# facebookresearch/visual_inertial_bundle_adjustment

Hardware: AMD Instinct MI355X
Metric: LM iterations/sec on 10k-pose/300k-landmark VI-BA (higher is better)
Workload: dtype f64; 1 GPU; config C: 5941186 obs, 300000 landmarks, 10000 rigs, reduced order 150483; rigs=10000, landmarks=300000, observations=5941186, parallelism=single GPU

## Files before the change

### visual_inertial_bundle_adjustment_amd/csrc/finalize.hip

```cpp
#include "host.hpp"

namespace viba_host {
namespace {

Knobs readKnobs(const vb_handle_s& h) {
  Knobs k;
  if (const char* e = getenv("VIBA_ND_CUTWIN")) k.cutWin = std::max(0.0, std::min(0.45, atof(e)));
  if (const char* e = getenv("VIBA_ND_LEAF")) k.leafDims = std::max<int64_t>(64, atoll(e));
  k.stats = getenv("VIBA_STATS") != nullptr;
  k.ptFuseMax = h.ptFuseMax, k.useSn = h.useSn, k.snStreams = h.snStreams;
  return k;
}

int uploadSched(const SchedHost& H, Sched& S) {
  static_cast<SchedShape&>(S) = H;
  if (upload(&S.potrfTileD, H.potrfTile) || upload(&S.potrfColD, H.potrfCol) || upload(&S.trsmDiagD, H.trsmDiag) ||
      upload(&S.trsmTargetD, H.trsmTarget) || upload(&S.trsmColD, H.trsmCol) || upload(&S.trsmRowD, H.trsmRow) ||
      upload(&S.updD, H.upd) || upload(&S.fanPairsD, H.fanPairs) || upload(&S.tasksFD, H.tasksF) ||
      upload(&S.tasksBD, H.tasksB) || upload(&S.expFD, H.expF) || upload(&S.expBD, H.expB) ||
      upload(&S.preReadyD, H.preReady) || upload(&S.ptfD, H.ptf) || upload(&S.ptfDiagD, H.ptfDiag))
    return VB_E_HIP;
  return 0;
}

int uploadSnSched(const SnSchedHost& H, SnSched& S) {
  static_cast<SnSchedShape&>(S) = H;
  if (upload(&S.updD, H.upd) || upload(&S.fanPairsD, H.fanPairs) || upload(&S.potD, H.pot) || upload(&S.rowD, H.row) ||
      upload(&S.fusD, H.fus) || upload(&S.copyD, H.copy) || upload(&S.invEarlyD, H.invEarly) ||
      upload(&S.invLateD, H.invLate))
    return VB_E_HIP;
  return 0;
}

void copyToHandle(vb_handle h, const Symbolic& A) {
  Dev& d = h->d;
  d.jac = makeJac(h->cfg.imu_calib_options);
  d.reproj = makeLoss(h->cfg.reproj_loss_radius, h->cfg.reproj_loss_cutoff);
  d.imu = makeLoss(h->cfg.imu_loss_radius, h->cfg.imu_loss_cutoff);
  d.T = TS;
  for (int k = 0; k < 9; k++) d.nvar[k] = A.reg.nvar[k];
  const int64_t nPts = A.reg.nPts;
  d.nRV = A.lay.nRV, d.nRed = A.lay.nRed, d.nPts = nPts, d.nT = A.lay.nT, d.nTiles = A.pat.nTiles;
  d.nObs = A.obs.nObs, d.nObsPad = A.obs.nObsPad, d.nYcol = A.pan.nYcol;
  d.nLxChunk = (int64_t)A.pan.lxChunk.size() / 3;
  d.lmB = A.shard.lmBegin, d.lmE = A.shard.lmEnd, d.root = A.shard.isRoot ? 1 : 0;
  d.nLmSmall = A.shard.nLmSmall, d.nLmBig = A.shard.nLmBig, d.lmBigCols = A.shard.lmBigCols;
  d.obB = A.shard.obB, d.obE = A.shard.obE, d.obFree = A.shard.obFree, d.fB = A.shard.fB, d.fE = A.shard.fE;
  d.nGroups = (int64_t)A.schur.grpRed.size() / 4;
  d.nTileWorks = (int64_t)A.schur.works.size();
  for (int fk = 1; fk < 14; fk++) {
    SmallFactors& sf = d.sf[fk];
    sf.nv = kNumVars[fk], sf.n = (int64_t)h->fint[fk].size(), sf.nc = A.small.nc[fk], sf.stage = A.small.stage[fk];
  }
  d.nSmallStage = A.small.nSmallStage;
  d.myRank = h->partRank, d.world = h->partWorld;
  d.nRS = h->nRS;

  h->rvKind = A.lay.rvKind, h->rvHandle = A.lay.rvHandle, h->rvDim = A.lay.rvDim, h->rvOff = A.lay.rvOff;
  h->lmOfPoint = A.reg.lmOfPoint;
  h->colOwner = A.lay.colOwner;
  h->nRedReal = A.lay.nRedReal, h->nParts = (int64_t)A.nd.partBegin.size();
  h->nParams = nPts + A.lay.nRV;
  h->order = nPts * 3 + A.lay.nRedReal;
  h->nPadRows = (int64_t)A.lay.padRows.size();
  h->nLmObs = A.obs.lmObs[nPts];
  h->lmBegin = A.shard.lmBegin, h->lmEnd = A.shard.lmEnd, h->isRoot = A.shard.isRoot;
  h->tileFill = A.pat.tileFill;
  h->colStart = A.pat.colStart, h->colTilesH = A.pat.colTiles, h->colRowsH = A.pat.colRows;
  h->rowStart = A.pat.rowStart, h->rowTilesH = A.pat.rowTiles, h->rowColH = A.pat.rowCol;
  h->nClear = (int64_t)A.schur.clearTiles.size();
  h->nTileEnt = (int64_t)A.schur.ents.size(), h->nObEnt = d.nGroups;
  h->tileFirst = A.schur.tileFirst, h->tileCount = A.schur.tileCount;
  h->shardTiles = A.schur.shardTiles;
  h->zeroRuns = A.part.zeroRuns, h->rootTiles = A.part.rootTiles, h->rootRows = A.part.rootRows;
  h->nOwnRows = (int64_t)A.part.ownRows.size();
  h->nLevels = A.pat.nLevels;
  h->nPairs = A.sch[0].nPairs + A.sch[1].nPairs;
  h->costRsB[0] = A.cost.rsBegin[0], h->costRsB[1] = A.cost.rsBegin[1];
  if (A.preint.present) h->piNoise = A.preint.noise;
}

int uploadRsTables(vb_handle h) {
  Dev& d = h->d;
  if (h->rsDevice) {
    const int64_t kWidenNs = 20000000;
    h->rsOff.assign(h->nRS + 1, 0);
    for (int32_t t = 0; t < h->nRS; t++) {
      const int64_t a = (h->rsMid[t] - h->rsHalf[t]) * 1000 - kWidenNs, b = (h->rsMid[t] + h->rsHalf[t]) * 1000 + kWidenNs;
      const int64_t cnt = std::upper_bound(h->imuT.begin(), h->imuT.end(), b) -
                          std::lower_bound(h->imuT.begin(), h->imuT.end(), a);
      h->rsOff[t + 1] = h->rsOff[t] + cnt + 4;
// ... 122 lines not shown
```

### visual_inertial_bundle_adjustment_amd/csrc/solver.hip

```cpp
#include "kernel_common.hpp"
#include <algorithm>
#include <string>

namespace viba {


template <int J>
__device__ __forceinline__ double rowbcast(double v) {
  return __builtin_amdgcn_mov_dpp(v, 0x150 + J, 0xF, 0xF, true);
}

__device__ __forceinline__ double rsqrt_nr(double x) {
  double y = __builtin_amdgcn_rsq(x);
  const double e = __builtin_fma(-(x * y), y, 1.0);
  return __builtin_fma(e * y, __builtin_fma(e, 0.375, 0.5), y);
}

template <int C, int J>
struct Upd16 {
  static __device__ __forceinline__ void run(double (&s)[16], double lc) {
    s[J] -= lc * rowbcast<J>(lc);
    Upd16<C, J + 1>::run(s, lc);
  }
};
template <int C>
struct Upd16<C, 16> {
  static __device__ __forceinline__ void run(double (&)[16], double) {}
};
template <int C>
struct Chol16 {
  static __device__ __forceinline__ void run(double (&s)[16], double (&invd)[16], int lane, bool& bad) {
    const double piv = rowbcast<C>(s[C]);
    bad |= !(piv > 0.0);
    const double y = rsqrt_nr(piv);
    invd[C] = y;
    const double lc = s[C] * y;
    s[C] = lc;
    Upd16<C, C + 1>::run(s, lc);
    Chol16<C + 1>::run(s, invd, lane, bad);
  }
};
template <>
struct Chol16<16> {
  static __device__ __forceinline__ void run(double (&)[16], double (&)[16], int, bool&) {}
};

template <int LDT = TS>
__device__ __forceinline__ void diag16(double* T, double* scratch, double* dinvS, int i, double4_t S, int lane,
                                       bool& bad) {
  const int lr = lane & 15, lq = lane >> 4;
#pragma unroll
  for (int r = 0; r < 4; r++) scratch[(lq + 4 * r) * 16 + lr] = S[r];
  __builtin_amdgcn_wave_barrier();
  double s[16], invd[16];
#pragma unroll
  for (int c = 0; c < 16; c++) s[c] = scratch[lr * 16 + c];
  Chol16<0>::run(s, invd, lane, bad);
  __builtin_amdgcn_wave_barrier();
  if (lane < 16) {
#pragma unroll
    for (int c = 0; c < 16; c++) {
      const double v = (c <= lane) ? s[c] : 0.0;
      scratch[lane * 16 + c] = v;
      T[(16 * i + c) * LDT + 16 * i + lane] = v;
    }
  }
  __builtin_amdgcn_fence(__ATOMIC_RELEASE, "wavefront");
  __builtin_amdgcn_wave_barrier();
  __builtin_amdgcn_fence(__ATOMIC_ACQUIRE, "wavefront");
  double acc[16];
#pragma unroll
  for (int r = 0; r < 16; r++) acc[r] = (r == lr) ? 1.0 : 0.0;
#pragma unroll
  for (int k = 0; k < 16; k++) {
    acc[k] *= invd[k];
#pragma unroll
    for (int r = k + 1; r < 16; r++) acc[r] -= scratch[r * 16 + k] * acc[k];
  }
  if (lane < 16) {
#pragma unroll
    for (int r = 0; r < 16; r++) dinvS[i * 256 + lane * 16 + r] = acc[r];
  }
  __builtin_amdgcn_wave_barrier();
}

__device__ __forceinline__ void lds_to_global(double* dst, const double* src, int n, int tid, int nthreads) {
  double* p = dst + tid;
  const double* q = src + tid;
#pragma unroll 8
  for (int i = tid; i < n; i += nthreads, p += nthreads, q += nthreads) *p = *q;
}

__device__ __forceinline__ void wave_sync_lds() {
  __builtin_amdgcn_fence(__ATOMIC_RELEASE, "wavefront");
  __builtin_amdgcn_wave_barrier();
  __builtin_amdgcn_fence(__ATOMIC_ACQUIRE, "wavefront");
}
__device__ __forceinline__ void potrf_forward(const Dev& d, const double* T, const double* dinvS, double* sh, int J,
                                              const double* bJ, double* y, int lane, bool store = true) {
  double br = bJ[lane];
#pragma unroll
  for (int i = 0; i < 4; i++) {
    sh[64 + lane] = br;
    wave_sync_lds();
    if ((lane >> 4) == i) {
      const int l = lane & 15;
      double v = 0.0;
#pragma unroll
      for (int m = 0; m < 16; m++) v += dinvS[i * 256 + m * 16 + l] * sh[64 + 16 * i + m];
      sh[16 * i + l] = v;
    }
    wave_sync_lds();
    if (i < 3) {
#pragma unroll
      for (int m = 0; m < 16; m++) br -= T[(16 * i + m) * TS + lane] * sh[16 * i + m];
    }
  }
  const int64_t row = (int64_t)J * TS + lane;
  if (store) y[row] = row < d.nRed ? sh[lane] : 0.0;
}

__device__ __forceinline__ void potrf4_core(const Dev& d, const double* A, double* T, double* scratch, double* dinvS,
                                            int tid) {
  const int lane = tid & 63, w = tid >> 6;
  const int lr = lane & 15, lq = lane >> 4;
  double4_t R[4];
#pragma unroll
  for (int j = 0; j < 4; j++) {
    if (j < w) {
#pragma unroll
      for (int r = 0; r < 4; r++) R[j][r] = A[(16 * j + lq + 4 * r) * TS + 16 * w + lr];
    } else if (j == w) {
#pragma unroll
      for (int r = 0; r < 4; r++) R[j][r] = A[(16 * w + lr) * TS + 16 * w + lq + 4 * r];
    } else {
#pragma unroll
      for (int r = 0; r < 4; r++) T[(16 * j + lq + 4 * r) * TS + 16 * w + lr] = 0.0;
    }
  }
  bool bad = false;
#pragma unroll
  for (int k = 0; k < 4; k++) {
    if (w == k) {
      diag16(T, scratch, dinvS, k, R[k], lane, bad);
    }
    __syncthreads();
    double4_t Lt = double4_t{0, 0, 0, 0};
    if (w > k) {
#pragma unroll
      for (int s = 0; s < 4; s++) Lt = mfma64(dinvS[k * 256 + (4 * s + lq) * 16 + lr], R[k][s], Lt);
#pragma unroll
      for (int r = 0; r < 4; r++) T[(16 * k + lq + 4 * r) * TS + 16 * w + lr] = Lt[r];
#pragma unroll
      for (int j = k + 1; j < 4; j++)
        if (j == w) {
#pragma unroll
          for (int s = 0; s < 4; s++) R[j] = mfma64(-Lt[s], Lt[s], R[j]);
        }
    }
    if (k < 2) {
      __syncthreads();
#pragma unroll
      for (int j = k + 1; j < 3; j++)
        if (j < w) {
#pragma unroll
          for (int s = 0; s < 4; s++) R[j] = mfma64(-T[(16 * k + 4 * s + lq) * TS + 16 * j + lr], Lt[s], R[j]);
        }
    }
  }
  __syncthreads();
  if (bad && lane == 0) atomicOr(d.err, 8);
}

__global__ void __launch_bounds__(256) potrf4_kernel(Dev d, const int32_t* tileList, const int32_t* cols,
                                                     double* dinvAll, const double* fwdB, double* fwdY) {
  __shared__ double T[TS * TS];
  __shared__ double scratch[256];
  __shared__ double dinvS[1024];
  const int tid = threadIdx.x, w = tid >> 6;
  double* A = d.tiles + (int64_t)tileList[blockIdx.x] * TS * TS;
  double* dinvG = dinvAll + (int64_t)cols[blockIdx.x] * 1024;
  potrf4_core(d, A, T, scratch, dinvS, tid);
  if (fwdB && w == 0) potrf_forward(d, T, dinvS, scratch, cols[blockIdx.x], fwdB + (int64_t)cols[blockIdx.x] * TS, fwdY, tid & 63);
  lds_to_global(A, T, TS * TS, tid, 256);
  lds_to_global(dinvG, dinvS, 1024, tid, 256);
}

__global__ void __launch_bounds__(256) potrf_trsm_kernel(Dev d, const int32_t* items, double* Lscr, double* dinvAll,
                                                         double* fwdB, double* fwdY) {
  __shared__ double T[TS * TS];
  __shared__ double scratch[256];
  __shared__ double dinvS[1024];
  const int32_t* it = items + 5 * (int64_t)blockIdx.x;
  const int32_t diagT = it[0], col = it[1], target = it[2], row = it[3], writer = it[4];
  const int tid = threadIdx.x, lane = tid & 63, w = tid >> 6;
  const int lr = lane & 15, lq = lane >> 4;
  double* At = target >= 0 ? d.tiles + (int64_t)target * TS * TS : nullptr;
  double av[4][4];
  if (At) {
#pragma unroll
    for (int k = 0; k < 4; k++)
#pragma unroll
      for (int r = 0; r < 4; r++) av[k][r] = At[(16 * k + lq + 4 * r) * TS + 16 * w + lr];
  }
  potrf4_core(d, d.tiles + (int64_t)diagT * TS * TS, T, scratch, dinvS, tid);
  if (fwdB && w == 0) potrf_forward(d, T, dinvS, scratch, col, fwdB + (int64_t)col * TS, fwdY, lane, writer != 0);
  if (writer) {
    lds_to_global(Lscr + (int64_t)col * TS * TS, T, TS * TS, tid, 256);
    lds_to_global(dinvAll + (int64_t)col * 1024, dinvS, 1024, tid, 256);
  }
  if (!At) return;
  __syncthreads();
  double4_t Xt[4];
#pragma unroll
  for (int k = 0; k < 4; k++) {
    double4_t acc = double4_t{av[k][0], av[k][1], av[k][2], av[k][3]};
#pragma unroll
    for (int k2 = 0; k2 < k; k2++)
#pragma unroll
      for (int s = 0; s < 4; s++) acc = mfma64(-T[(16 * k2 + 4 * s + lq) * TS + 16 * k + lr], Xt[k2][s], acc);
    double4_t res = double4_t{0, 0, 0, 0};
#pragma unroll
    for (int s = 0; s < 4; s++) res = mfma64(dinvS[k * 256 + (4 * s + lq) * 16 + lr], acc[s], res);
    Xt[k] = res;
  }
#pragma unroll
  for (int k = 0; k < 4; k++)
// ... 29 lines not shown
  for (int k = 0; k < 4; k++) {
    double4_t a = acc[k];
#pragma unroll
    for (int k2 = 0; k2 < k; k2++)
#pragma unroll
      for (int s = 0; s < 4; s++) a = mfma64(-lv[k * (k - 1) / 2 + k2][s], Xt[k2][s], a);
    double4_t res = double4_t{0, 0, 0, 0};
#pragma unroll
    for (int s = 0; s < 4; s++) res = mfma64(dv[k][s], a[s], res);
    Xt[k] = res;
  }
}
template <int LD = TS>
__device__ __forceinline__ void gemm_nt_sub(const double* M, const double4_t (&Xt)[4], double4_t (&acc)[4], int lr, int lq,
                                            int kmax = 3) {
#pragma unroll
  for (int k = 0; k < 4; k++) {
    if (k > kmax) break;
    double mv[4][4];
#pragma unroll
    for (int k2 = 0; k2 < 4; k2++)
#pragma unroll
      for (int s = 0; s < 4; s++) mv[k2][s] = M[(16 * k2 + 4 * s + lq) * LD + 16 * k + lr];
#pragma unroll
    for (int k2 = 0; k2 < 4; k2++)
#pragma unroll
      for (int s = 0; s < 4; s++) acc[k] = mfma64(-mv[k2][s], Xt[k2][s], acc[k]);
  }
}
__device__ __forceinline__ void load_rows(const double* A, double4_t (&acc)[4], int w, int lr, int lq) {
#pragma unroll
  for (int k = 0; k < 4; k++)
#pragma unroll
    for (int r = 0; r < 4; r++) acc[k][r] = A[(16 * k + lq + 4 * r) * TS + 16 * w + lr];
}
__device__ __forceinline__ void store_rows(double* A, const double4_t (&X)[4], int w, int lr, int lq) {
#pragma unroll
  for (int k = 0; k < 4; k++)
#pragma unroll
    for (int r = 0; r < 4; r++) A[(16 * k + lq + 4 * r) * TS + 16 * w + lr] = X[k][r];
}
__device__ __forceinline__ double rows_dot(const double4_t (&X)[4], const double* y, int lq) {
  double v = 0.0;
#pragma unroll
  for (int k = 0; k < 4; k++)
#pragma unroll
    for (int r = 0; r < 4; r++) v += X[k][r] * y[16 * k + lq + 4 * r];
  v += __shfl_xor(v, 16, 64);
  v += __shfl_xor(v, 32, 64);
  return v;
}

template <int NB, int LDT>
__device__ __forceinline__ void potrf_core(const Dev& d, const double* A11, const double* A21, const double* A22,
                                           double* T, double* scratch, double* dinvS, int tid,
                                           const double* b0 = nullptr, const double* b1 = nullptr,
                                           double* yb = nullptr) {
  const int lane = tid & 63, w = tid >> 6;
  const int lr = lane & 15, lq = lane >> 4;
  double bw = 0.0;
  if (b0 && w < NB) bw = (w < 4 ? b0 : b1)[16 * (w & 3) + lr];
  double4_t R[NB];
  if (w < NB) {
#pragma unroll
    for (int j = 0; j < NB; j++) {
      const double* P = w < 4 ? A11 : (j < 4 ? A21 : A22);
      const int rr = 16 * (w & 3), cc = 16 * (j & 3);
      if (j < w) {
#pragma unroll
        for (int r = 0; r < 4; r++) R[j][r] = P[(cc + lq + 4 * r) * TS + rr + lr];
      } else if (j == w) {
#pragma unroll
        for (int r = 0; r < 4; r++) R[j][r] = P[(cc + lr) * TS + rr + lq + 4 * r];
      } else {
#pragma unroll
        for (int r = 0; r < 4; r++) T[(16 * j + lq + 4 * r) * LDT + 16 * w + lr] = 0.0;
      }
    }
  }
  bool bad = false;
#pragma unroll
  for (int k = 0; k < NB; k++) {
    if (w == k) {
      diag16<LDT>(T, scratch, dinvS, k, R[k], lane, bad);
      if (b0) {
        if (lq == 0) yb[16 * k + lr] = bw;
        wave_sync_lds();
        if (lq == 0) {
          double v = 0.0;
#pragma unroll
          for (int m = 0; m < 16; m++) v += dinvS[k * 256 + m * 16 + lr] * yb[16 * k + m];
          yb[128 + 16 * k + lr] = v;
        }
      }
    }
    __syncthreads();
    double4_t Lt = double4_t{0, 0, 0, 0};
    if (w > k && w < NB) {
#pragma unroll
      for (int s = 0; s < 4; s++) Lt = mfma64(dinvS[k * 256 + (4 * s + lq) * 16 + lr], R[k][s], Lt);
#pragma unroll
      for (int r = 0; r < 4; r++) T[(16 * k + lq + 4 * r) * LDT + 16 * w + lr] = Lt[r];
      if (b0) {
        double v = 0.0;
#pragma unroll
        for (int r = 0; r < 4; r++) v += Lt[r] * yb[128 + 16 * k + lq + 4 * r];
        v += __shfl_xor(v, 16, 64);
        v += __shfl_xor(v, 32, 64);
        bw -= v;
      }
#pragma unroll
      for (int j = k + 1; j < NB; j++)
        if (j == w) {
#pragma unroll
          for (int s = 0; s < 4; s++) R[j] = mfma64(-Lt[s], Lt[s], R[j]);
        }
    }
    if (k < NB - 2) {
      __syncthreads();
#pragma unroll
      for (int j = k + 1; j < NB - 1; j++)
        if (j < w && w < NB) {
#pragma unroll
          for (int s = 0; s < 4; s++) R[j] = mfma64(-T[(16 * k + 4 * s + lq) * LDT + 16 * j + lr], Lt[s], R[j]);
        }
    }
  }
  __syncthreads();
  if (bad && lane == 0) atomicOr(d.err, 8);
}

template <int NB, int LDT>
__device__ __forceinline__ void trsm_lds(const double* T, const double* dinvS, const double4_t (&a)[NB], double4_t (&X)[NB],
                                         int lr, int lq) {
#pragma unroll
  for (int k = 0; k < NB; k++) {
    double4_t acc = a[k];
#pragma unroll
    for (int k2 = 0; k2 < k; k2++)
#pragma unroll
      for (int s = 0; s < 4; s++) acc = mfma64(-T[(16 * k2 + 4 * s + lq) * LDT + 16 * k + lr], X[k2][s], acc);
    double4_t res = double4_t{0, 0, 0, 0};
#pragma unroll
    for (int s = 0; s < 4; s++) res = mfma64(dinvS[k * 256 + (4 * s + lq) * 16 + lr], acc[s], res);
    X[k] = res;
  }
}

template <int NB, int LDT>
__device__ __forceinline__ void store_block_tiles(double* L11, double* L21, double* L22, const double* T, int tid,
                                                  int nthreads) {
  for (int i = tid; i < (16 * NB) * (16 * NB); i += nthreads) {
    const int col = i / (16 * NB), row = i % (16 * NB);
    if (row < 64 && col >= 64) continue;
    double* P = row < 64 ? L11 : (col < 64 ? L21 : L22);
    P[(col & 63) * TS + (row & 63)] = T[col * LDT + row];
  }
}

__global__ void __launch_bounds__(512) snpotrf8_kernel(Dev d, const int32_t* items, double* dinvAll, const double* fwdB,
                                                       double* fwdY) {
  __shared__ double T[128 * 128];
  __shared__ double scratch[256];
  __shared__ double dinvS[8 * 256];
  __shared__ double yb[256];
  const int32_t* it = items + 4 * (int64_t)blockIdx.x;
  const int32_t t11 = it[0], J = it[1], t21 = it[2], t22 = it[3];
  const int tid = threadIdx.x, lane = tid & 63, w = tid >> 6;
  double* A11 = d.tiles + (int64_t)t11 * TS * TS;
  if (t21 < 0) {
    potrf_core<4, 128>(d, A11, nullptr, nullptr, T, scratch, dinvS, tid, fwdB ? fwdB + (int64_t)J * TS : nullptr,
                       nullptr, yb);
    if (fwdB && w == 0) {
      const int64_t row = (int64_t)J * TS + lane;
      fwdY[row] = row < d.nRed ? yb[128 + lane] : 0.0;
    }
    store_block_tiles<4, 128>(A11, nullptr, nullptr, T, tid, 512);
    for (int i = tid; i < 1024; i += 512) dinvAll[(int64_t)J * 1024 + i] = dinvS[i];
    return;
  }
  double* A21 = d.tiles + (int64_t)t21 * TS * TS;
  double* A22 = d.tiles + (int64_t)t22 * TS * TS;
  potrf_core<8, 128>(d, A11, A21, A22, T, scratch, dinvS, tid, fwdB ? fwdB + (int64_t)J * TS : nullptr,
                     fwdB ? fwdB + (int64_t)(J + 1) * TS : nullptr, yb);
  if (fwdB && w < 2) {
    const int64_t row = (int64_t)(J + w) * TS + lane;
    fwdY[row] = row < d.nRed ? yb[128 + 64 * w + lane] : 0.0;
  }
  store_block_tiles<8, 128>(A11, A21, A22, T, tid, 512);
  for (int i = tid; i < 2048; i += 512) dinvAll[(int64_t)J * 1024 + i] = dinvS[i];
}

__global__ void __launch_bounds__(512) snpotrf_trsm8_kernel(Dev d, const int32_t* items, double* Lscr, double* dinvAll,
                                                            double* fwdB, double* fwdY) {
  __shared__ double T[128 * 128];
  __shared__ double scratch[256];
  __shared__ double dinvS[8 * 256];
  __shared__ double yb[256];
  const int32_t* it = items + 8 * xcd_block(blockIdx.x, gridDim.x);
  const int32_t t11 = it[0], J = it[1], t21 = it[2], t22 = it[3], tI1 = it[4], tI2 = it[5], I = it[6], writer = it[7];
  const int tid = threadIdx.x, lane = tid & 63, w = tid >> 6;
  const int lr = lane & 15, lq = lane >> 4;
  const bool two = t21 >= 0;
  const int64_t nT = d.nT;
  const double* A11 = d.tiles + (int64_t)t11 * TS * TS;
  const double* b0 = fwdB ? fwdB + (int64_t)J * TS : nullptr;
  if (two)
    potrf_core<8, 128>(d, A11, d.tiles + (int64_t)t21 * TS * TS, d.tiles + (int64_t)t22 * TS * TS, T, scratch, dinvS, tid,
                       b0, fwdB ? fwdB + (int64_t)(J + 1) * TS : nullptr, yb);
  else
    potrf_core<4, 128>(d, A11, nullptr, nullptr, T, scratch, dinvS, tid, b0, nullptr, yb);
  double4_t a[8];
  if (I >= 0 && w < 4) {
#pragma unroll
    for (int k = 0; k < 8; k++) {
      const int32_t t = k < 4 ? tI1 : tI2;
      if (t >= 0 && (k < 4 || two)) {
#pragma unroll
        for (int r = 0; r < 4; r++) a[k][r] = d.tiles[(int64_t)t * TS * TS + (16 * (k & 3) + lq + 4 * r) * TS + 16 * w + lr];
      } else {
        a[k] = double4_t{0, 0, 0, 0};
      }
    }
  }
  if (fwdB && writer && w < (two ? 2 : 1)) {
    const int64_t row = (int64_t)(J + w) * TS + lane;
    fwdY[row] = row < d.nRed ? yb[128 + 64 * w + lane] : 0.0;
  }
  if (writer) {
    if (two) store_block_tiles<8, 128>(Lscr + J * TS * TS, Lscr + (nT + J) * TS * TS, Lscr + (J + 1) * TS * TS, T, tid, 512);
    else store_block_tiles<4, 128>(Lscr + J * TS * TS, nullptr, nullptr, T, tid, 512);
    for (int i = tid; i < (two ? 2048 : 1024); i += 512) dinvAll[(int64_t)J * 1024 + i] = dinvS[i];
  }
  if (I < 0) return;
  if (w >= 4) return;
  double v = 0.0;
  if (two) {
    double4_t X[8];
    trsm_lds<8, 128>(T, dinvS, a, X, lr, lq);
#pragma unroll
    for (int k = 0; k < 8; k++) {
      const int32_t t = k < 4 ? tI1 : tI2;
      if (t >= 0) {
#pragma unroll
        for (int r = 0; r < 4; r++) d.tiles[(int64_t)t * TS * TS + (16 * (k & 3) + lq + 4 * r) * TS + 16 * w + lr] = X[k][r];
      }
#pragma unroll
      for (int r = 0; r < 4; r++) v += X[k][r] * yb[128 + 16 * k + lq + 4 * r];
    }
  } else {
    double4_t a4[4], X[4];
#pragma unroll
    for (int k = 0; k < 4; k++) a4[k] = a[k];
    trsm_lds<4, 128>(T, dinvS, a4, X, lr, lq);
    store_rows(d.tiles + (int64_t)tI1 * TS * TS, X, w, lr, lq);
#pragma unroll
    for (int k = 0; k < 4; k++)
#pragma unroll
      for (int r = 0; r < 4; r++) v += X[k][r] * yb[128 + 16 * k + lq + 4 * r];
  }
  if (fwdB) {
    v += __shfl_xor(v, 16, 64);
    v += __shfl_xor(v, 32, 64);
    if (lq == 0) atomicAdd(fwdB + (int64_t)I * TS + 16 * w + lr, -v);
  }
}

__device__ __forceinline__ void sntrsm_body(const Dev& d, const int32_t* items, const double* dinvAll, const double* fwdY,
                                            double* fwdB) {
  const int32_t* it = items + 8 * xcd_block(blockIdx.x, gridDim.x);
  const int32_t tI1 = it[0], tI2 = it[1], J = it[2], J2 = it[3], I = it[4], t11 = it[5], t21 = it[6], t22 = it[7];
  const int lane = threadIdx.x & 63, w = threadIdx.x >> 6;
// ... 624 lines not shown
```

### visual_inertial_bundle_adjustment_amd/csrc/symbolic.hip

```cpp
#include "symbolic.hpp"

namespace viba_host {

void psdSqrt(const double* Pm, int m, double* U) {
  std::vector<double> A(Pm, Pm + m * m), V(m * m, 0.0);
  for (int i = 0; i < m; i++) V[i * m + i] = 1.0;
  for (int sweep = 0; sweep < 60; sweep++) {
    double off = 0;
    for (int p = 0; p < m; p++)
      for (int q = p + 1; q < m; q++) off += A[p * m + q] * A[p * m + q];
    if (off < 1e-30) break;
    for (int p = 0; p < m; p++)
      for (int q = p + 1; q < m; q++) {
        const double apq = A[p * m + q];
        if (std::abs(apq) < 1e-300) continue;
        const double th = 0.5 * (A[q * m + q] - A[p * m + p]) / apq;
        const double t = (th >= 0 ? 1.0 : -1.0) / (std::abs(th) + std::sqrt(th * th + 1.0));
        const double c = 1.0 / std::sqrt(t * t + 1.0), s = t * c;
        for (int k = 0; k < m; k++) {
          const double akp = A[k * m + p], akq = A[k * m + q];
          A[k * m + p] = c * akp - s * akq, A[k * m + q] = s * akp + c * akq;
        }
        for (int k = 0; k < m; k++) {
          const double apk = A[p * m + k], aqk = A[q * m + k];
// ... 1084 lines not shown

namespace {
void pairColumns(const Pattern& pat, const std::vector<int8_t>& colOwner, int32_t nT, const Select& sel,
                 std::vector<int8_t>& role) {
  role.assign(nT, 0);
  for (int32_t J = 0; J + 1 < nT; J++) {
    if (role[J]) continue;
    const int64_t a = pat.colStart[J], b = pat.colStart[J + 1], a2 = pat.colStart[J + 1], b2 = pat.colStart[J + 2];
    if (b - a < 2 || pat.colRows[a + 1] != J + 1 || colOwner[J] != colOwner[J + 1] || !sel.col[J] || !sel.col[J + 1])
      continue;
    bool subset = true;
    int64_t q = a2 + 1;
    for (int64_t c = a + 2; c < b && subset; c++) {
      while (q < b2 && pat.colRows[q] < pat.colRows[c]) q++;
      subset = q < b2 && pat.colRows[q] == pat.colRows[c];
    }
    if (subset) role[J] = 1, role[J + 1] = 2;
  }
}

void assignStreams(const Pattern& pat, int32_t nT, const std::vector<int8_t>& role, const std::vector<int64_t>& start,
                   int nStreams, bool stats, std::vector<int32_t>& stream, std::vector<int32_t>& parent) {
  std::vector<int32_t> snOf(nT);
  std::vector<double> weight(nT, 0.0);
  std::vector<std::vector<int32_t>> kids(nT);
  for (int32_t J = 0; J < nT; J++) snOf[J] = role[J] == 2 ? J - 1 : J;
  for (int32_t J0 = 0; J0 < nT; J0++) {
    if (role[J0] == 2) continue;
    const int32_t Jl = role[J0] == 1 ? J0 + 1 : J0;
    if (pat.colStart[Jl + 1] - pat.colStart[Jl] > 1) parent[J0] = snOf[pat.colRows[pat.colStart[Jl] + 1]];
    for (int32_t J = J0; J <= Jl; J++) weight[J0] += (double)contributionsInto(pat, start, J);
  }
  std::vector<double> own(weight);
  for (int32_t J0 = 0; J0 < nT; J0++)
    if (role[J0] != 2 && parent[J0] >= 0) weight[parent[J0]] += weight[J0], kids[parent[J0]].push_back(J0);
  std::vector<int32_t> front;
  for (int32_t J0 = 0; J0 < nT; J0++)
    if (role[J0] != 2 && parent[J0] < 0) front.push_back(J0);
  std::vector<int8_t> top(nT, 0);
  for (int it = 0; it < 4 * nT && front.size() < 256; it++) {
    double tot = 0.0;
    size_t xi = 0;
    for (size_t i = 0; i < front.size(); i++) {
      tot += weight[front[i]];
      if (weight[front[i]] > weight[front[xi]]) xi = i;
    }
    const int32_t X = front[xi];
    if (weight[X] <= 1.15 * tot / nStreams || kids[X].empty()) break;
    top[X] = 1;
    front.erase(front.begin() + (ptrdiff_t)xi);
    front.insert(front.end(), kids[X].begin(), kids[X].end());
  }
  std::stable_sort(front.begin(), front.end(), [&](int32_t a, int32_t b) { return weight[a] > weight[b]; });
  std::vector<double> load(nStreams, 0.0);
  std::vector<int32_t> rootStream(nT, -1);
  for (int32_t X : front) {
    const int g = (int)(std::min_element(load.begin(), load.end()) - load.begin());
    load[g] += weight[X], rootStream[X] = g;
  }
  for (int32_t J0 = nT - 1; J0 >= 0; J0--)
    if (role[J0] != 2 && !top[J0]) stream[J0] = rootStream[J0] >= 0 ? rootStream[J0] : parent[J0] >= 0 ? stream[parent[J0]] : 0;
  for (int32_t J0 = 0; J0 < nT; J0++)
    if (role[J0] != 2 && top[J0]) {
      int32_t best = -1;
      for (int32_t C : kids[J0])
        if (best < 0 || weight[C] > weight[best]) best = C;
      stream[J0] = best >= 0 ? stream[best] : 0;
    }
  for (int32_t J0 = 0; J0 < nT; J0++)
    if (role[J0] == 1) stream[J0 + 1] = stream[J0];
  if (stats) {
    std::vector<double> gw(nStreams, 0.0), gt(nStreams, 0.0);
    std::vector<int> gs(nStreams, 0);
    for (int32_t J0 = 0; J0 < nT; J0++)
      if (role[J0] != 2) gw[stream[J0]] += own[J0], gs[stream[J0]]++, gt[stream[J0]] += top[J0] ? own[J0] : 0.0;
    for (int g = 0; g < nStreams; g++)
      fprintf(stderr, "[factor stats] stream %d: supernodes %d, contributions %.0f (%.0f above the cut)\n", g, gs[g], gw[g],
              gt[g]);
  }
}
}

Status supernodeSchedule(const Pattern& pat, const std::vector<int8_t>& colOwner, int32_t nT, const Select& sel,
                         int nStreams, bool stats, SnSchedHost& S) {
  std::vector<int8_t>& role = S.pairRole;
  pairColumns(pat, colOwner, nT, sel, role);
  std::vector<int32_t>& lev = S.level;
  lev.assign(nT, 0);
  int32_t nLev = 0;
  for (int32_t J = 0; J < nT; J++) {
    if (role[J] == 2) continue;
    int32_t lv = 0;
    for (int32_t X = J; X <= J + (role[J] == 1 ? 1 : 0); X++)
      for (int64_t i = pat.rowStart[X]; i < pat.rowStart[X + 1]; i++) {
        const int32_t K = pat.rowCol[i];
        if (X == J + 1 && K == J) continue;
        lv = std::max(lv, lev[K] + 1);
      }
    lev[J] = lv;
    if (role[J] == 1) lev[J + 1] = lv;
    nLev = std::max(nLev, lv + 1);
  }
  std::vector<std::vector<int32_t>> sup(nLev);
  for (int32_t J = 0; J < nT; J++)
    if (role[J] != 2) sup[lev[J]].push_back(J);
  std::vector<int32_t> sources;
  for (int32_t L = 0; L < nLev; L++)
    for (int32_t J0 : sup[L])
      for (int32_t K = J0; K <= J0 + (role[J0] == 1 ? 1 : 0); K++) sources.push_back(K);
  std::vector<int64_t> start;
  if (Status e = fanInPairs(pat, nT, sel, sources, &role, start, S.fanPairs)) return e;
  std::vector<int32_t>& stream = S.stream;
  stream.assign(nT, 0);
  std::vector<int32_t> parent(nT, -1);
  const int G = std::max(1, nStreams);
  if (G > 1) assignStreams(pat, nT, role, start, G, stats, stream, parent);
  std::vector<int> nActive(nLev, 0);
  for (int32_t L = 0; L < nLev; L++) {
    uint32_t m = 0;
    for (int32_t J0 : sup[L]) m |= 1u << stream[J0];
    nActive[L] = __builtin_popcount(m);
  }
  const int64_t fuseMax = 256;
  const int64_t fanTarget = 3072;
  S.upd.clear(), S.pot.clear(), S.row.clear(), S.fus.clear(), S.copy.clear();
  S.lvU.assign(1, 0), S.lvS.assign(1, 0), S.lvR.assign(1, 0), S.lvF.assign(1, 0);
  S.segG.clear(), S.segL.clear(), S.segDep.clear();
  S.nTwo = 0;
  auto tile = [&](int32_t I, int32_t J) { return pat.tileIdx[(size_t)I * nT + J]; };
  for (int32_t L = 0; L < nLev; L++)
    for (int g = 0; g < G; g++) {
      std::vector<int32_t> supL;
      uint32_t dep = 0;
      for (int32_t J0 : sup[L])
        if (stream[J0] == g) supL.push_back(J0);
      if (supL.empty()) continue;
      if (G > 1)
        for (int32_t J0 = 0; J0 < nT; J0++)
          if (role[J0] != 2 && parent[J0] >= 0 && stream[parent[J0]] == g && lev[parent[J0]] == L && stream[J0] != g)
            dep |= 1u << stream[J0];
      int64_t total = 0;
      for (int32_t J0 : supL)
        for (int32_t J = J0; J <= J0 + (role[J0] == 1 ? 1 : 0); J++) total += contributionsInto(pat, start, J);
      const int share = std::max(1, nActive[L]);
      const int64_t fanWgs = fanTarget / share;
      const int64_t chunk = std::min<int64_t>(32, std::max<int64_t>(4, (total + fanWgs - 1) / fanWgs));
      const size_t firstChunk = S.upd.size() / 4;
      int64_t nRowsL = 0;
      for (int32_t J0 : supL) {
        if (!sel.col[J0]) continue;
        const int32_t Jl = role[J0] == 1 ? J0 + 1 : J0;
        nRowsL += pat.colStart[Jl + 1] - pat.colStart[Jl] - 1;
      }
      const bool fused = nRowsL <= fuseMax / share;
      for (int32_t J0 : supL) {
        const bool two = role[J0] == 1;
        const int32_t J2 = two ? J0 + 1 : -1;
        for (int32_t J = J0; J <= (two ? J2 : J0); J++)
          for (int64_t c = pat.colStart[J]; c < pat.colStart[J + 1]; c++)
            if (sel.tgt[J]) fanChunks(pat.colTiles[c], start, chunk, S.upd);
        if (!sel.col[J0]) continue;
        const int32_t t11 = tile(J0, J0), t21 = two ? tile(J2, J0) : -1, t22 = two ? tile(J2, J2) : -1;
        S.nTwo += two ? 1 : 0;
        const int32_t Jl = two ? J2 : J0;
        const int64_t r0 = pat.colStart[Jl] + 1, r1 = pat.colStart[Jl + 1];
        if (fused) {
          S.copy.insert(S.copy.end(), {t11, J0});
          if (two) S.copy.insert(S.copy.end(), {t22, J2, t21, nT + J0});
          if (r1 == r0) S.fus.insert(S.fus.end(), {t11, J0, t21, t22, -1, -1, -1, 1});
          for (int64_t c = r0; c < r1; c++) {
            const int32_t I = pat.colRows[c];
            S.fus.insert(S.fus.end(), {t11, J0, t21, t22, two ? tile(I, J0) : pat.colTiles[c], two ? pat.colTiles[c] : -1, I,
                                       c == r0 ? 1 : 0});
          }
          continue;
        }
        S.pot.insert(S.pot.end(), {t11, J0, t21, t22});
        for (int64_t c = r0; c < r1; c++) {
          const int32_t I = pat.colRows[c];
          S.row.insert(S.row.end(), {two ? tile(I, J0) : pat.colTiles[c], two ? pat.colTiles[c] : -1, J0, J2, I, t11, t21, t22});
        }
      }
      sortChunksPerXcd(S.upd, firstChunk);
      S.lvU.push_back((int64_t)S.upd.size() / 4), S.lvS.push_back((int64_t)S.pot.size() / 4);
      S.lvR.push_back((int64_t)S.row.size() / 8), S.lvF.push_back((int64_t)S.fus.size() / 8);
      S.segG.push_back(g), S.segL.push_back(L), S.segDep.push_back((int32_t)dep);
    }
  S.nGroups = G;
  S.nLevels = nLev, S.nPairs = start[pat.nTiles];
  S.nSuper = 0;
  for (int32_t J = 0; J < nT; J++) S.nSuper += (role[J] != 2 && sel.col[J]) ? 1 : 0;
  S.nCopy = (int64_t)S.copy.size() / 2;
  S.invEarly.clear(), S.invLate.clear();
  const int nSeg = (int)S.segG.size();
  int chain0 = 0;
  for (int i = 1; i < nSeg; i++)
    if (S.segL[i] == S.segL[i - 1]) chain0 = i + 1;
  std::vector<uint8_t> early(nT, 0);
  for (int i = 0; i < chain0; i++)
    for (int64_t k = S.lvS[i]; k < S.lvS[i + 1]; k++) {
      early[S.pot[4 * k + 1]] = 1;
      if (S.pot[4 * k + 2] >= 0) early[S.pot[4 * k + 1] + 1] = 1;
    }
  for (int32_t J = 0; J < nT; J++)
    if (sel.col[J]) (early[J] ? S.invEarly : S.invLate).push_back(J);
  S.nInvEarly = (int64_t)S.invEarly.size(), S.nInvLate = (int64_t)S.invLate.size();
// ... 38 lines not shown
      }
    }
    small.stage[fk] = small.nSmallStage;
    small.nSmallStage += n;
  }
  return {};
}

Status preintInputs(const Input& in, PreintInputs& preint) {
  preint.present = !in.piSrc.empty();
  if (!preint.present) return {};
  const int nStreams = (int)std::max<size_t>(1, in.piT.size());
  preint.off.assign(nStreams + 1, 0);
  preint.t.clear(), preint.v.clear();
  for (int s = 0; s < nStreams; s++) {
    const std::vector<int64_t>& t = s == 0 ? in.imuT : in.piT[s];
    const std::vector<double>& v = s == 0 ? in.imuV : in.piV[s];
    preint.t.insert(preint.t.end(), t.begin(), t.end());
    preint.v.insert(preint.v.end(), v.begin(), v.end());
    preint.off[s + 1] = (int64_t)preint.t.size();
  }
  for (const PreintSrc& p : in.piSrc)
    if (p.imu < 0 || p.imu >= nStreams || preint.off[p.imu + 1] == preint.off[p.imu])
      return {VB_E_ARG, "preintegration source names an IMU without a measurement stream"};
  preint.noise.assign((size_t)nStreams * 6, 0.0);
  for (int s = 0; s < nStreams; s++)
    for (int k = 0; k < 6; k++)
      preint.noise[s * 6 + k] = 6 * s + k < (int)in.piNoise.size() ? in.piNoise[6 * s + k] : kDefaultImuNoise[k];
  return {};
}

void costOrder(const Layout& lay, const Observations& obs, const Shard& shard, CostOrder& cost) {
  const int64_t nObs = obs.nObs;
  cost.order.assign(nObs, 0);
  std::vector<int64_t> cuts = {0, shard.obB, shard.obE, shard.fB, shard.fE, nObs};
  std::sort(cuts.begin(), cuts.end());
  for (size_t c = 0; c + 1 < cuts.size(); c++) {
    int64_t w = cuts[c];
    for (int pass = 0; pass < 2; pass++)
      for (int64_t i = cuts[c]; i < cuts[c + 1]; i++)
        if ((obs.obRS[i] >= 0) == (pass == 1)) cost.order[w++] = (int32_t)i;
  }
  auto rsStart = [&](int64_t b, int64_t e) {
    int64_t n = 0;
    for (int64_t i = b; i < e; i++) n += obs.obRS[i] < 0;
    return b + n;
  };
  cost.rsBegin[0] = rsStart(shard.obB, shard.obE), cost.rsBegin[1] = rsStart(shard.fB, shard.fE);
  cost.pack.assign((size_t)nObs * 8, 0);
  cost.cp.assign((size_t)nObs * 6, 0.0);
  for (int64_t i = 0; i < nObs; i++) {
    const int32_t o = cost.order[i];
    int32_t* q = &cost.pack[(size_t)i * 8];
    q[0] = o, q[1] = obs.obPt[o], q[2] = obs.obPose[o], q[3] = obs.obExtr[o], q[4] = obs.obIntr[o], q[5] = obs.obRS[o];
    q[6] = obs.obVel[o];
    q[7] = (obs.obRed[(size_t)o * 4 + kSlotIntr] >= 0 ? 1 : 0) | (obs.obRed[(size_t)o * 4 + kSlotVel] >= 0 ? 2 : 0);
    for (int k = 0; k < 6; k++) cost.cp[(size_t)i * 6 + k] = obs.obC[(size_t)o * 6 + k];
  }
}

Status analyze(const Input& in, Symbolic& S) {
  if (Status e = registerVariables(in, S.reg)) return e;
  timeOrder(in, S.reg, S.time);
  dissect(in, S.reg, S.time, S.nd);
  if (Status e = reducedLayout(S.reg, S.nd, S.lay)) return e;
  S.lmRank.assign(S.reg.nPts, 0);
  if (in.partSet) landmarkOwners(in, S.lay, S.reg, S.lmRank);
  if (Status e = sortObservations(in, S.reg, S.lay, S.obs)) return e;
  if (Status e = landmarkPanels(S.reg, S.lay, S.obs, S.pan)) return e;
  if (Status e = shardRanges(in, S.lay, S.lmRank, S.obs, S.pan, S.shard)) return e;
  tilePattern(in, S.lay, S.obs, S.pan, S.pat);
  if (Status e = schurWork(in, S.lay, S.obs, S.pan, S.shard, S.pat, S.schur)) return e;
  if (in.knobs.stats) printFactorStats(S.pat, S.lay.nT);
  const int32_t nT = S.lay.nT;
  const bool rootToo = in.partSet && in.partRank == 0;
  const Select sel0 = in.partSet ? selectRank(S.lay.colOwner, in.partRank, in.partWorld) : selectAll(nT);
  const Select sel1 = selectRoot(S.lay.colOwner, in.partWorld);
  if (Status e = columnSchedule(S.pat, nT, sel0, in.knobs.ptFuseMax, S.sch[0])) return e;
  if (rootToo)
    if (Status e = columnSchedule(S.pat, nT, sel1, in.knobs.ptFuseMax, S.sch[1])) return e;
  if (in.partSet) partitionSets(S.lay, S.pat, in.partRank, in.partWorld, S.part);
  if (in.knobs.useSn) {
    const int streams = in.partSet ? 1 : in.knobs.snStreams;
    if (Status e = supernodeSchedule(S.pat, S.lay.colOwner, nT, sel0, streams, in.knobs.stats, S.sn[0])) return e;
    if (rootToo)
      if (Status e = supernodeSchedule(S.pat, S.lay.colOwner, nT, sel1, 1, in.knobs.stats, S.sn[1])) return e;
  }
  if (Status e = smallConstants(in, S.small)) return e;
  if (Status e = preintInputs(in, S.preint)) return e;
  costOrder(S.lay, S.obs, S.shard, S.cost);
  return {};
}

}
```

### visual_inertial_bundle_adjustment_amd/csrc/symbolic.hpp

```cpp
#pragma once
#include <algorithm>
#include <array>
#include <climits>
#include <cmath>
#include <cstdint>
#include <cstdio>
#include <numeric>
#include <string>
#include <utility>
#include <vector>

#include "../../include/viba_hip.h"
#include "engine.hpp"

namespace viba_host {
using namespace viba;

constexpr int TS = 64;
constexpr int kVarData[9] = {3, 7, 3, 3, 24, 7, 32, 7, 4};
constexpr int kNumVars[14] = {5, 6, 9, 10, 2, 2, 2, 2, 2, 1, 1, 1, 1, 1};
constexpr int kNumConsts[14] = {6, 331, 331, 331, 4, 23, 17, 6, 6, 43, 55, 41, 13, 13};
constexpr double kDefaultImuNoise[6] = {6.6297049e-3, 6.6297049e-3, 6.6297049e-3, 2.7415568e-05, 2.7415568e-05, 2.7415568e-05};
const int kFK[14][10] = {{0, 1, 5, 4, 2}, {6, 1, 2, 1, 2, 8}, {6, 1, 2, 3, 1, 2, 3, 7, 8},
                         {6, 1, 2, 3, 7, 1, 2, 3, 7, 8}, {3, 7}, {6, 6}, {4, 4}, {7, 7}, {5, 5}, {1}, {6}, {4},
                         {5}, {7}};

inline ImuIdx makeJac(int mask) {
  ImuIdx J;
  int i = 0;
  J.gB = (mask & 1) ? (i += 3) - 3 : -1;
  J.aB = (mask & 2) ? (i += 3) - 3 : -1;
  J.gS = (mask & 4) ? (i += 3) - 3 : -1;
  J.aS = (mask & 8) ? (i += 3) - 3 : -1;
  J.gN = (mask & 16) ? (i += 6) - 6 : -1;
  J.aN = (mask & 32) ? (i += 3) - 3 : -1;
  J.rT = (mask & 64) ? (i += 1) - 1 : -1;
  J.gaT = (mask & 128) ? (i += 1) - 1 : -1;
  J.size = i;
  return J;
}

void psdSqrt(const double* Pm, int m, double* U);
bool precisionChol(const double* cov, int m, double* U);

struct Knobs {
  double cutWin = 0.05;
  int64_t leafDims = 1024;
  int64_t ptFuseMax = 256;
  bool useSn = true;
  int snStreams = 2;
  bool stats = false;
};

struct Input {
  const std::vector<double> (&data)[9];
  const std::vector<uint8_t> (&cst)[9];
  const std::vector<int32_t> (&fvars)[14];
  const std::vector<int32_t> (&fint)[14];
  const std::vector<double> (&fconst)[14];
  int imuCalibOptions;
  int32_t nRS;
  bool sharded;
  int64_t lmBegin, lmEnd;
  bool isRoot;
  bool partSet;
  int partRank, partWorld;
  const std::vector<PreintSrc>& piSrc;
  const std::vector<int64_t>& imuT;
  const std::vector<double>& imuV;
  const std::vector<std::vector<int64_t>>& piT;
  const std::vector<std::vector<double>>& piV;
  const std::vector<double>& piNoise;
  Knobs knobs;
};

struct Status {
  int code = 0;
  const char* msg = "";
  explicit operator bool() const { return code != 0; }
};

struct Registration {
  int64_t nvar[9] = {};
  std::vector<std::pair<int, int>> reg;
  std::vector<int32_t> regOf[9];
  std::vector<int> tdims;
  std::vector<int32_t> lmOfPoint;
  int64_t nPts = 0;
  int jacSize = 0;
};
struct TimeOrder {
  std::vector<int> order;
  std::vector<int> pos;
  std::vector<int> hiP, loP;
};
struct Dissection {
  std::vector<int> order;
  std::vector<size_t> partBegin;
  std::vector<int> partOwner;
};
struct Layout {
  int32_t nRV = 0, nT = 0;
  int64_t nRed = 0, nRedReal = 0;
  std::vector<int32_t> rvKind, rvHandle, rvDim;
  std::vector<int64_t> rvOff;
  std::vector<int32_t> redOf[9];
  std::vector<int64_t> padRows;
  std::vector<int8_t> colOwner;
};
struct Observations {
  int64_t nObs = 0, nObsPad = 0;
  std::vector<int64_t> perm;
  std::vector<int32_t> obPose, obExtr, obIntr, obVel, obRS, obPt;
  std::vector<int32_t> obRed;
  std::vector<double> obC;
  std::vector<int64_t> lmObs;
};
struct Panels {
  std::vector<int64_t> lmBlk, lmY;
  std::vector<int32_t> blkRed, blkCol, obCol, pcRow, pcBlk, bxEnt;
  std::vector<int64_t> bxStart;
  std::vector<int64_t> oxStart, lxStart, lxChunk;
  std::vector<int32_t> oxObs, oxSlot, lxLm, lxCol;
  int64_t nYcol = 0;
};
struct Shard {
  int64_t lmBegin = 0, lmEnd = 0;
  bool isRoot = true;
  int64_t obB = 0, obE = 0, obFree = 0, fB = 0, fE = 0;
  std::vector<int32_t> lmList;
  int64_t nLmSmall = 0, nLmBig = 0;
  int32_t lmBigCols = 0;
};
// ... 31 lines not shown
  int32_t nLevels = 0;
  int64_t nPairs = 0;
  int64_t nF = 0, nB = 0, nPreReady = 0;
  bool built = false;
};
struct SchedHost : SchedShape {
  std::vector<int32_t> potrfTile, potrfCol, trsmDiag, trsmTarget, trsmCol, trsmRow, upd, fanPairs;
  std::vector<int32_t> tasksF, tasksB, expF, expB, preReady, ptf, ptfDiag;
};
struct SnSchedShape {
  int32_t nLevels = 0;
  int64_t nPairs = 0;
  int64_t nSuper = 0, nTwo = 0;
  std::vector<int64_t> lvU, lvS, lvR;
  std::vector<int32_t> segG, segL, segDep;
  int nGroups = 1;
  std::vector<int64_t> lvF;
  int64_t nCopy = 0;
  int64_t nInvEarly = 0, nInvLate = 0;
  bool built = false;
};
struct SnSchedHost : SnSchedShape {
  std::vector<int32_t> upd, fanPairs, pot, row, fus, copy, invEarly, invLate;
  std::vector<int8_t> pairRole;
  std::vector<int32_t> level, stream;
};
struct PartitionSets {
  std::vector<std::pair<int64_t, int64_t>> zeroRuns;
  std::vector<int32_t> rootTiles, rootRows, ownRows;
};
struct SmallConsts {
  int nc[14] = {};
  int64_t stage[14] = {};
  std::vector<double> consts[14];
  int64_t nSmallStage = 0;
};
struct PreintInputs {
  bool present = false;
  std::vector<int64_t> off, t;
  std::vector<double> v, noise;
};
struct CostOrder {
  std::vector<int32_t> order, pack;
  std::vector<double> cp;
  int64_t rsBegin[2] = {0, 0};
};

struct Symbolic {
  Registration reg;
  TimeOrder time;
  Dissection nd;
  Layout lay;
  std::vector<int> lmRank;
  Observations obs;
  Panels pan;
  Shard shard;
  Pattern pat;
  SchurWork schur;
  SchedHost sch[2];
  SnSchedHost sn[2];
  PartitionSets part;
  SmallConsts small;
  PreintInputs preint;
  CostOrder cost;
};

Status registerVariables(const Input& in, Registration& reg);
void timeOrder(const Input& in, const Registration& reg, TimeOrder& time);
void dissect(const Input& in, const Registration& reg, const TimeOrder& time, Dissection& nd);
Status reducedLayout(const Registration& reg, const Dissection& nd, Layout& lay);
void landmarkOwners(const Input& in, const Layout& lay, Registration& reg, std::vector<int>& lmRank);
Status sortObservations(const Input& in, const Registration& reg, const Layout& lay, Observations& obs);
Status landmarkPanels(const Registration& reg, const Layout& lay, const Observations& obs, Panels& pan);
Status shardRanges(const Input& in, const Layout& lay, const std::vector<int>& lmRank, const Observations& obs,
                   const Panels& pan, Shard& shard);
void tilePattern(const Input& in, const Layout& lay, const Observations& obs, const Panels& pan, Pattern& pat);
Status schurWork(const Input& in, const Layout& lay, const Observations& obs, const Panels& pan, const Shard& shard,
                 const Pattern& pat, SchurWork& schur);
Select selectAll(int32_t nT);
Select selectRank(const std::vector<int8_t>& colOwner, int rank, int world);
Select selectRoot(const std::vector<int8_t>& colOwner, int world);
Status columnSchedule(const Pattern& pat, int32_t nT, const Select& sel, int64_t ptFuseMax, SchedHost& S);
Status supernodeSchedule(const Pattern& pat, const std::vector<int8_t>& colOwner, int32_t nT, const Select& sel,
                         int nStreams, bool stats, SnSchedHost& S);
void partitionSets(const Layout& lay, const Pattern& pat, int rank, int world, PartitionSets& part);
Status smallConstants(const Input& in, SmallConsts& small);
Status preintInputs(const Input& in, PreintInputs& preint);
void costOrder(const Layout& lay, const Observations& obs, const Shard& shard, CostOrder& cost);

Status analyze(const Input& in, Symbolic& S);

}
```

Measured before the change: 57.35 LM iterations/s.

## Factor supernode panels directly in global tiles with a small LDS panel buffer

The supernode POTRF kernel no longer stages the whole 128x128 block in a 128 KB LDS array and copies it back afterwards. Each wave is specialised at compile time to its column, reads and writes its tiles in global memory, and shares only the current 16-row panel through a 16x128 LDS buffer. This removes the bulk LDS staging and the final store pass and sharply cuts LDS use, which could allow more blocks per CU, at the cost of more global-memory traffic during the factorisation. The supernode fuse limit also becomes configurable through an environment variable, with the same default of 256.

```diff
diff --git a/visual_inertial_bundle_adjustment_amd/csrc/finalize.hip b/visual_inertial_bundle_adjustment_amd/csrc/finalize.hip
--- a/visual_inertial_bundle_adjustment_amd/csrc/finalize.hip
+++ b/visual_inertial_bundle_adjustment_amd/csrc/finalize.hip
@@ -7,6 +7,7 @@
   Knobs k;
   if (const char* e = getenv("VIBA_ND_CUTWIN")) k.cutWin = std::max(0.0, std::min(0.45, atof(e)));
   if (const char* e = getenv("VIBA_ND_LEAF")) k.leafDims = std::max<int64_t>(64, atoll(e));
+  if (const char* e = getenv("VIBA_SN_FUSE_MAX")) k.snFuseMax = std::max<int64_t>(0, atoll(e));
   k.stats = getenv("VIBA_STATS") != nullptr;
   k.ptFuseMax = h.ptFuseMax, k.useSn = h.useSn, k.snStreams = h.snStreams;
   return k;
diff --git a/visual_inertial_bundle_adjustment_amd/csrc/solver.hip b/visual_inertial_bundle_adjustment_amd/csrc/solver.hip
--- a/visual_inertial_bundle_adjustment_amd/csrc/solver.hip
+++ b/visual_inertial_bundle_adjustment_amd/csrc/solver.hip
@@ -45,8 +45,8 @@
   static __device__ __forceinline__ void run(double (&)[16], double (&)[16], int, bool&) {}
 };
 
-template <int LDT = TS>
-__device__ __forceinline__ void diag16(double* T, double* scratch, double* dinvS, int i, double4_t S, int lane,
+template <int LDO = TS>
+__device__ __forceinline__ void diag16(double* Lout, double* scratch, double* dinvS, int i, double4_t S, int lane,
                                        bool& bad) {
   const int lr = lane & 15, lq = lane >> 4;
 #pragma unroll
@@ -62,7 +62,7 @@
     for (int c = 0; c < 16; c++) {
       const double v = (c <= lane) ? s[c] : 0.0;
       scratch[lane * 16 + c] = v;
-      T[(16 * i + c) * LDT + 16 * i + lane] = v;
+      Lout[c * LDO + lane] = v;
     }
   }
   __builtin_amdgcn_fence(__ATOMIC_RELEASE, "wavefront");
@@ -142,7 +142,7 @@
 #pragma unroll
   for (int k = 0; k < 4; k++) {
     if (w == k) {
-      diag16(T, scratch, dinvS, k, R[k], lane, bad);
+      diag16(T + (16 * k) * TS + 16 * k, scratch, dinvS, k, R[k], lane, bad);
     }
     __syncthreads();
     double4_t Lt = double4_t{0, 0, 0, 0};
@@ -338,7 +338,7 @@
 #pragma unroll
   for (int k = 0; k < NB; k++) {
     if (w == k) {
-      diag16<LDT>(T, scratch, dinvS, k, R[k], lane, bad);
+      diag16<LDT>(T + (16 * k) * LDT + 16 * k, scratch, dinvS, k, R[k], lane, bad);
       if (b0) {
         if (lq == 0) yb[16 * k + lr] = bw;
         wave_sync_lds();
@@ -383,6 +383,110 @@
     }
   }
   __syncthreads();
+  if (bad && lane == 0) atomicOr(d.err, 8);
+}
+
+struct BlockTiles {
+  double *P11, *P21, *P22;
+  __device__ __forceinline__ double* at(int w, int j) const {
+    return (w < 4 ? P11 : (j < 4 ? P21 : P22)) + (16 * (j & 3)) * TS + 16 * (w & 3);
+  }
+};
+template <int NB, int W>
+__device__ __forceinline__ void potrf_panel_wave(const BlockTiles& A, double* Pn, double* scratch, double* dinvS, int lane,
+                                                 const double* b0, const double* b1, double* yb, bool& bad) {
+  const int lr = lane & 15, lq = lane >> 4;
+  if constexpr (W >= NB) {
+#pragma unroll
+    for (int k = 0; k < 2 * NB - 1; k++) __syncthreads();
+  } else {
+    double bw = 0.0;
+    if (b0) bw = (W < 4 ? b0 : b1)[16 * (W & 3) + lr];
+    double4_t R[W + 1];
+#pragma unroll
+    for (int j = 0; j < W; j++) {
+      const double* P = A.at(W, j);
+#pragma unroll
+      for (int r = 0; r < 4; r++) R[j][r] = P[(lq + 4 * r) * TS + lr];
+    }
+    {
+      const double* P = A.at(W, W);
+#pragma unroll
+      for (int r = 0; r < 4; r++) R[W][r] = P[lr * TS + lq + 4 * r];
+    }
+#pragma unroll
+    for (int j = W + 1; j < NB; j++)
+      if (j < 4 || W >= 4) {
+        double* Z = A.at(W, j);
+#pragma unroll
+        for (int r = 0; r < 4; r++) Z[(lq + 4 * r) * TS + lr] = 0.0;
+      }
+#pragma unroll
+    for (int k = 0; k < NB; k++) {
+      if (k == W) {
+        diag16<TS>(A.at(W, W), scratch, dinvS, W, R[W], lane, bad);
+        if (b0) {
+          if (lq == 0) yb[16 * k + lr] = bw;
+          wave_sync_lds();
+          if (lq == 0) {
+            double v = 0.0;
+#pragma unroll
+            for (int m = 0; m < 16; m++) v += dinvS[k * 256 + m * 16 + lr] * yb[16 * k + m];
+            yb[128 + 16 * k + lr] = v;
+          }
+        }
+      }
+      __syncthreads();
+      double4_t Lt = double4_t{0, 0, 0, 0};
+      if (k < W) {
+#pragma unroll
+        for (int s = 0; s < 4; s++) Lt = mfma64(dinvS[k * 256 + (4 * s + lq) * 16 + lr], R[k][s], Lt);
+        if (k < NB - 2) {
+#pragma unroll
+          for (int r = 0; r < 4; r++) Pn[(lq + 4 * r) * 128 + 16 * W + lr] = Lt[r];
+        }
+        double* G = A.at(W, k);
+#pragma unroll
+        for (int r = 0; r < 4; r++) G[(lq + 4 * r) * TS + lr] = Lt[r];
+        if (b0) {
+          double v = 0.0;
+#pragma unroll
+          for (int r = 0; r < 4; r++) v += Lt[r] * yb[128 + 16 * k + lq + 4 * r];
+          v += __shfl_xor(v, 16, 64);
+          v += __shfl_xor(v, 32, 64);
+          bw -= v;
+        }
+#pragma unroll
+        for (int s = 0; s < 4; s++) R[W] = mfma64(-Lt[s], Lt[s], R[W]);
+      }
+      if (k < NB - 2) {
+        __syncthreads();
+#pragma unroll
+        for (int j = k + 1; j < NB - 1; j++)
+          if (j < W) {
+#pragma unroll
+            for (int s = 0; s < 4; s++) R[j] = mfma64(-Pn[(4 * s + lq) * 128 + 16 * j + lr], Lt[s], R[j]);
+          }
+      }
+    }
+    __syncthreads();
+  }
+}
+template <int NB>
+__device__ __forceinline__ void potrf_panel(const Dev& d, const BlockTiles& A, double* Pn, double* scratch, double* dinvS,
+                                            int tid, const double* b0, const double* b1, double* yb) {
+  const int lane = tid & 63;
+  bool bad = false;
+  switch (__builtin_amdgcn_readfirstlane(tid >> 6)) {
+    case 0: potrf_panel_wave<NB, 0>(A, Pn, scratch, dinvS, lane, b0, b1, yb, bad); break;
+    case 1: potrf_panel_wave<NB, 1>(A, Pn, scratch, dinvS, lane, b0, b1, yb, bad); break;
+    case 2: potrf_panel_wave<NB, 2>(A, Pn, scratch, dinvS, lane, b0, b1, yb, bad); break;
+    case 3: potrf_panel_wave<NB, 3>(A, Pn, scratch, dinvS, lane, b0, b1, yb, bad); break;
+    case 4: potrf_panel_wave<NB, 4>(A, Pn, scratch, dinvS, lane, b0, b1, yb, bad); break;
+    case 5: potrf_panel_wave<NB, 5>(A, Pn, scratch, dinvS, lane, b0, b1, yb, bad); break;
+    case 6: potrf_panel_wave<NB, 6>(A, Pn, scratch, dinvS, lane, b0, b1, yb, bad); break;
+    default: potrf_panel_wave<NB, 7>(A, Pn, scratch, dinvS, lane, b0, b1, yb, bad); break;
+  }
   if (bad && lane == 0) atomicOr(d.err, 8);
 }
 
@@ -416,7 +520,7 @@
 
 __global__ void __launch_bounds__(512) snpotrf8_kernel(Dev d, const int32_t* items, double* dinvAll, const double* fwdB,
                                                        double* fwdY) {
-  __shared__ double T[128 * 128];
+  __shared__ double Pn[16 * 128];
   __shared__ double scratch[256];
   __shared__ double dinvS[8 * 256];
   __shared__ double yb[256];
@@ -425,25 +529,23 @@
   const int tid = threadIdx.x, lane = tid & 63, w = tid >> 6;
   double* A11 = d.tiles + (int64_t)t11 * TS * TS;
   if (t21 < 0) {
-    potrf_core<4, 128>(d, A11, nullptr, nullptr, T, scratch, dinvS, tid, fwdB ? fwdB + (int64_t)J * TS : nullptr,
-                       nullptr, yb);
+    potrf_panel<4>(d, BlockTiles{A11, nullptr, nullptr}, Pn, scratch, dinvS, tid, fwdB ? fwdB + (int64_t)J * TS : nullptr,
+                   nullptr, yb);
     if (fwdB && w == 0) {
       const int64_t row = (int64_t)J * TS + lane;
       fwdY[row] = row < d.nRed ? yb[128 + lane] : 0.0;
     }
-    store_block_tiles<4, 128>(A11, nullptr, nullptr, T, tid, 512);
     for (int i = tid; i < 1024; i += 512) dinvAll[(int64_t)J * 1024 + i] = dinvS[i];
     return;
   }
   double* A21 = d.tiles + (int64_t)t21 * TS * TS;
   double* A22 = d.tiles + (int64_t)t22 * TS * TS;
-  potrf_core<8, 128>(d, A11, A21, A22, T, scratch, dinvS, tid, fwdB ? fwdB + (int64_t)J * TS : nullptr,
-                     fwdB ? fwdB + (int64_t)(J + 1) * TS : nullptr, yb);
+  potrf_panel<8>(d, BlockTiles{A11, A21, A22}, Pn, scratch, dinvS, tid, fwdB ? fwdB + (int64_t)J * TS : nullptr,
+                 fwdB ? fwdB + (int64_t)(J + 1) * TS : nullptr, yb);
   if (fwdB && w < 2) {
     const int64_t row = (int64_t)(J + w) * TS + lane;
     fwdY[row] = row < d.nRed ? yb[128 + 64 * w + lane] : 0.0;
   }
-  store_block_tiles<8, 128>(A11, A21, A22, T, tid, 512);
   for (int i = tid; i < 2048; i += 512) dinvAll[(int64_t)J * 1024 + i] = dinvS[i];
 }
 
diff --git a/visual_inertial_bundle_adjustment_amd/csrc/symbolic.hip b/visual_inertial_bundle_adjustment_amd/csrc/symbolic.hip
--- a/visual_inertial_bundle_adjustment_amd/csrc/symbolic.hip
+++ b/visual_inertial_bundle_adjustment_amd/csrc/symbolic.hip
@@ -1190,7 +1190,7 @@
 }
 
 Status supernodeSchedule(const Pattern& pat, const std::vector<int8_t>& colOwner, int32_t nT, const Select& sel,
-                         int nStreams, bool stats, SnSchedHost& S) {
+                         int nStreams, int64_t fuseMax, bool stats, SnSchedHost& S) {
   std::vector<int8_t>& role = S.pairRole;
   pairColumns(pat, colOwner, nT, sel, role);
   std::vector<int32_t>& lev = S.level;
@@ -1229,7 +1229,6 @@
     for (int32_t J0 : sup[L]) m |= 1u << stream[J0];
     nActive[L] = __builtin_popcount(m);
   }
-  const int64_t fuseMax = 256;
   const int64_t fanTarget = 3072;
   S.upd.clear(), S.pot.clear(), S.row.clear(), S.fus.clear(), S.copy.clear();
   S.lvU.assign(1, 0), S.lvS.assign(1, 0), S.lvR.assign(1, 0), S.lvF.assign(1, 0);
@@ -1434,9 +1433,9 @@
   if (in.partSet) partitionSets(S.lay, S.pat, in.partRank, in.partWorld, S.part);
   if (in.knobs.useSn) {
     const int streams = in.partSet ? 1 : in.knobs.snStreams;
-    if (Status e = supernodeSchedule(S.pat, S.lay.colOwner, nT, sel0, streams, in.knobs.stats, S.sn[0])) return e;
+    if (Status e = supernodeSchedule(S.pat, S.lay.colOwner, nT, sel0, streams, in.knobs.snFuseMax, in.knobs.stats, S.sn[0])) return e;
     if (rootToo)
-      if (Status e = supernodeSchedule(S.pat, S.lay.colOwner, nT, sel1, 1, in.knobs.stats, S.sn[1])) return e;
+      if (Status e = supernodeSchedule(S.pat, S.lay.colOwner, nT, sel1, 1, in.knobs.snFuseMax, in.knobs.stats, S.sn[1])) return e;
   }
   if (Status e = smallConstants(in, S.small)) return e;
   if (Status e = preintInputs(in, S.preint)) return e;
diff --git a/visual_inertial_bundle_adjustment_amd/csrc/symbolic.hpp b/visual_inertial_bundle_adjustment_amd/csrc/symbolic.hpp
--- a/visual_inertial_bundle_adjustment_amd/csrc/symbolic.hpp
+++ b/visual_inertial_bundle_adjustment_amd/csrc/symbolic.hpp
@@ -49,6 +49,7 @@
   int64_t ptFuseMax = 256;
   bool useSn = true;
   int snStreams = 2;
+  int64_t snFuseMax = 256;
   bool stats = false;
 };
 
@@ -246,7 +247,7 @@
 Select selectRoot(const std::vector<int8_t>& colOwner, int world);
 Status columnSchedule(const Pattern& pat, int32_t nT, const Select& sel, int64_t ptFuseMax, SchedHost& S);
 Status supernodeSchedule(const Pattern& pat, const std::vector<int8_t>& colOwner, int32_t nT, const Select& sel,
-                         int nStreams, bool stats, SnSchedHost& S);
+                         int nStreams, int64_t fuseMax, bool stats, SnSchedHost& S);
 void partitionSets(const Layout& lay, const Pattern& pat, int rank, int world, PartitionSets& part);
 Status smallConstants(const Input& in, SmallConsts& small);
 Status preintInputs(const Input& in, PreintInputs& preint);
```

New measurement: 57.86 LM iterations/s, median of 6. No clear change (+0.9%).
